# 1879615351/Go-RIO

Hardware: AMD Instinct MI355X
Metric: APD-GICP GN iters/sec on 16k-pt scans + GP-preint windows/sec (higher is better)
Workload: dtype f32 search / f64 accumulate; 1 GPU; C4: 64 scan pairs 16384x16384 + 64 GP windows 1 s @ 200 Hz per GPU, k-NN covariances + 20 fixed GN iterations per pair; pairs_per_gpu=64, target_points=16384, optimizer=GN (convergence test disabled), search=pruned, parallelism=batch shard x1 (no collective)

## Files before the change

go-rio_amd/apd.py:

```python
import ctypes as C
import os

import numpy as np

REG_NONE, REG_MIN_EIG, REG_NORMALIZED_MIN_EIG, REG_PLANE, REG_FROBENIUS = range(5)
OPT_GAUSS_NEWTON, OPT_LEVENBERG_MARQUARDT = 0, 1
SEARCH_BRUTE_FORCE, SEARCH_PRUNED = 0, 1


class GorioError(RuntimeError):
    def __init__(self, code, msg):
        super().__init__(f"gorio error {code}: {msg}")
        self.code = code


class ApdParams(C.Structure):

    _fields_ = [
        ("k_correspondences", C.c_int),
        ("regularization", C.c_int),
        ("dist_var", C.c_double),
        ("azimuth_var", C.c_double),
        ("elevation_var", C.c_double),
        ("corr_dist_threshold", C.c_double),
        ("max_iterations", C.c_int),
        ("rotation_epsilon", C.c_double),
        ("transformation_epsilon", C.c_double),
        ("optimizer", C.c_int),
        ("lm_max_iterations", C.c_int),
        ("lm_init_lambda_factor", C.c_double),
        ("search", C.c_int),
        ("cl_weight_points", C.c_int),
        ("keep_knn_indices", C.c_int),
    ]


APD_SYMBOLS = [
    "gorio_apd_create", "gorio_apd_destroy", "gorio_apd_last_error", "gorio_apd_default_params", "gorio_apd_set_params",
    "gorio_apd_get_params", "gorio_apd_set_source", "gorio_apd_set_target", "gorio_apd_set_source_device",
    "gorio_apd_set_target_device", "gorio_apd_set_clouds_device_batch", "gorio_apd_clear_source", "gorio_apd_clear_target", "gorio_apd_swap_source_and_target",
    "gorio_apd_set_source_covariances", "gorio_apd_set_target_covariances", "gorio_apd_get_source_covariances",
    "gorio_apd_get_target_covariances", "gorio_apd_calculate_covariances", "gorio_apd_get_knn_indices", "gorio_apd_align",
    "gorio_apd_align_batch", "gorio_apd_linearize", "gorio_apd_compute_error", "gorio_apd_get_correspondences",
    "gorio_apd_get_mahalanobis", "gorio_apd_transform_source", "gorio_apd_fitness_score", "gorio_apd_fitness_score_batch", "gorio_apd_set_profiling",
    "gorio_apd_get_stage_times", "gorio_apd_set_target_shared", "gorio_comm_get_unique_id", "gorio_apd_comm_init", "gorio_apd_comm_destroy", "gorio_apd_comm_info", "gorio_apd_debug_set_shard", "gorio_apd_debug_set_schedule", "gorio_apd_set_target_submap", "gorio_apd_get_target_points",
    "gorio_apd_set_method", "gorio_apd_get_method", "gorio_apd_get_voxelmap", "gorio_apd_get_voxel_correspondences",
]

METHOD_APDGICP, METHOD_GICP, METHOD_VGICP = 0, 1, 2
VOXEL_DIRECT27, VOXEL_DIRECT7, VOXEL_DIRECT1, VOXEL_DIRECT_RADIUS = 0, 1, 2, 3
VOXEL_ADDITIVE, VOXEL_ADDITIVE_WEIGHTED, VOXEL_MULTIPLICATIVE = 0, 1, 2
VOXEL_OFFSETS = {VOXEL_DIRECT27: 27, VOXEL_DIRECT7: 7, VOXEL_DIRECT1: 1}

_lib = None


def load_library():
    global _lib
    if _lib is None:
        from . import LIB_PATH

        if not os.path.exists(LIB_PATH):
            raise GorioError(-2, f"{LIB_PATH} is missing: run __graft_entry__.build() (no CPU fallback exists)")
        _lib = C.CDLL(LIB_PATH)
        _lib.gorio_apd_last_error.restype = C.c_char_p
    return _lib


def _p(a, t):
    return C.cast(a.__array_interface__["data"][0], C.POINTER(t))


def _check(h, rc):
    if rc < 0:
        msg = load_library().gorio_apd_last_error(h)
        raise GorioError(rc, msg.decode() if msg else "")
    return rc

# ... 189 lines not shown

    def clearTarget(self):
        _check(self._h, self._lib.gorio_apd_clear_target(self._h))
        self._n_tgt = 0

    def swapSourceAndTarget(self):
        _check(self._h, self._lib.gorio_apd_swap_source_and_target(self._h))
        self._n_src, self._n_tgt = self._n_tgt, self._n_src

    def setSourceCovariances(self, cov):
        cov = np.ascontiguousarray(cov, np.float64).reshape(-1, 16)
        _check(self._h, self._lib.gorio_apd_set_source_covariances(self._h, _p(cov, C.c_double), cov.shape[0]))

    def setTargetCovariances(self, cov):
        cov = np.ascontiguousarray(cov, np.float64).reshape(-1, 16)
        _check(self._h, self._lib.gorio_apd_set_target_covariances(self._h, _p(cov, C.c_double), cov.shape[0]))

    def _get_covs(self, fn, n):
        cnt = _check(self._h, fn(self._h, None, 0))
        out = np.zeros((cnt, 4, 4), np.float64)
        if cnt:
            _check(self._h, fn(self._h, _p(out, C.c_double), cnt))
        return out

    def getSourceCovariances(self):
        return self._get_covs(self._lib.gorio_apd_get_source_covariances, self._n_src)

    def getTargetCovariances(self):
        return self._get_covs(self._lib.gorio_apd_get_target_covariances, self._n_tgt)

    def calculateCovariances(self):
        _check(self._h, self._lib.gorio_apd_calculate_covariances(self._h))

    def getKnnIndices(self, which):
        n = self._n_src if which == 0 else self._n_tgt
        k = self.params.k_correspondences
        idx = np.empty((n, k), np.int32)
        _check(self._h, self._lib.gorio_apd_get_knn_indices(self._h, int(which), _p(idx, C.c_int), n * k))
        return idx

    def align(self, guess=None):
        g = np.ascontiguousarray(np.eye(4) if guess is None else guess, np.float32)
        T = np.zeros((4, 4), np.float32)
        H = np.zeros((6, 6), np.float64)
        conv, nit, nlin = C.c_int(0), C.c_int(0), C.c_int(0)
        _check(self._h, self._lib.gorio_apd_align(self._h, _p(g, C.c_float), _p(T, C.c_float), _p(H, C.c_double), C.byref(conv), C.byref(nit), C.byref(nlin)))
        self._final = T
        self._converged = bool(conv.value)
        return dict(T=T, H=H, converged=bool(conv.value), nr_iterations=nit.value, n_linearize=nlin.value)

    def hasConverged(self):
        return self._converged

    def getFinalTransformation(self):
        return self._final

    def linearize(self, T):
        T = np.ascontiguousarray(T, np.float64)
        H = np.zeros((6, 6), np.float64)
        b = np.zeros(6, np.float64)
        err = C.c_double(0.0)
        _check(self._h, self._lib.gorio_apd_linearize(self._h, _p(T, C.c_double), _p(H, C.c_double), _p(b, C.c_double), C.byref(err)))
        return err.value, H, b

    def evaluateCost(self, relative_pose):
        return self.linearize(np.asarray(relative_pose, np.float32).astype(np.float64))
# ... 112 lines not shown
```

go-rio_amd/csrc/apd_api.hip:

```cpp
#include <hip/hip_runtime.h>
#include <dlfcn.h>
#include <rccl/rccl.h>

#include <cfloat>
#include <climits>
#include <cmath>
#include <cstdio>
#include <cstdlib>
#include <cstring>
#include <memory>
#include <mutex>
#include <string>
#include <unordered_set>
#include <vector>

#include "../../include/gorio_apd.h"
#include "apd_kernels.hip"
#include "apd_index.hip"
#include "apd_submap.hip"
#include "apd_voxel.hip"
#include "apd_prep.hip"
#include "../../include/gorio_prep.h"
#include "apd_ground.hip"
#include "../../include/gorio_sc.h"
#include "apd_sc.hip"

using namespace gorio;

namespace {

constexpr int kPad = 16;
constexpr float kFar = 1e30f;

struct DevCloud {
  float *x = nullptr, *y = nullptr, *z = nullptr, *label = nullptr;
  float4* p4 = nullptr;
  double *cov6 = nullptr, *geo_w = nullptr;
  int* knn = nullptr;
  int* redo = nullptr;
  float* kth = nullptr;
  int redo_cap = 0;
  float* part_d = nullptr;
  int* part_i = nullptr;
  size_t part_cap = 0;
  int knn_k = 0;
  bool knn_valid = false;
  int n = 0, n_pad = 0, cap = 0;
  bool present = false;
  int cov_count = 0;
  int cov_k = -1, cov_reg = -1;
  SearchIndex idx = SearchIndex{nullptr, nullptr, nullptr, nullptr, nullptr, nullptr, nullptr, nullptr, 0, 0, 0, 0};
  unsigned long long* keys = nullptr;
  unsigned int* bb = nullptr;
  int idx_cap = 0, keys_cap = 0;
  bool idx_valid = false;
  unsigned long long* vm_keys = nullptr;
  int vm_keys_cap = 0;
  int* vm_counts = nullptr;
  int vm_counts_cap = 0;
  int* vm_bb = nullptr;
  IndexJob* vm_job = nullptr;
  unsigned long long* vm_vkey = nullptr;
  double* vm_mean = nullptr;
  double* vm_cov6 = nullptr;
  int* vm_num = nullptr;
  int vm_cap = 0, vm_nv = 0;
  int vm_min[3] = {0, 0, 0}, vm_dim[3] = {0, 0, 0};
  double vm_res = 0.0;
  bool vm_mult = false;
  bool vm_valid = false;
  VoxelMapView voxel_view() const { return VoxelMapView{vm_vkey, vm_mean, vm_cov6, vm_num, vm_nv, {vm_min[0], vm_min[1], vm_min[2]}, {vm_dim[0], vm_dim[1], vm_dim[2]}, vm_res}; }
  int device = 0;
  CloudView view() const { return CloudView{x, y, z, label, p4, cov6, geo_w, n, n_pad, idx}; }
  DevCloud() = default;
  DevCloud(const DevCloud&) = delete;
  DevCloud& operator=(const DevCloud&) = delete;
  ~DevCloud();
};

}

struct gorio_apd {
  int device = 0;
  hipStream_t stream = nullptr;
  gorio_apd_params params;
  std::shared_ptr<DevCloud> src, tgt;
  unsigned long long* best_key = nullptr;
  int* seed = nullptr;
// ... 393 lines not shown
      HIP_TRY(h, hipMalloc(&c.idx.s4, sizeof(float4) * cap));
      HIP_TRY(h, hipMalloc(&c.idx.tbox, sizeof(float) * 8 * (cap / 32)));
      HIP_TRY(h, hipMalloc(&c.idx.sbox, sizeof(float) * 8 * (cap / 512)));
      HIP_TRY(h, hipMalloc(&c.idx.bbox, sizeof(float) * 8 * (cap / 32768 + 1)));
      c.idx_cap = cap;
    }
    if (npow2 > c.keys_cap) {
      hipFree(c.keys);
      c.keys = nullptr;
      HIP_TRY(h, hipMalloc(&c.keys, sizeof(unsigned long long) * npow2));
      c.keys_cap = npow2;
    }
    if (!c.bb) HIP_TRY(h, hipMalloc(&c.bb, sizeof(unsigned int) * 6));
    c.idx.n = c.n;
    c.idx.n_spad = n_spad;
    c.idx.n_tiles = n_spad / 32;
    c.idx.n_super = n_spad / 512;
    IndexJob& j = jobs[q];
    j.x = c.x; j.y = c.y; j.z = c.z; j.n = c.n; j.npow2 = npow2; j.keys = c.keys; j.bb = c.bb; j.idx = c.idx;
    max_pow2 = std::max(max_pow2, npow2);
    max_spad = std::max(max_spad, n_spad);
    max_n = std::max(max_n, c.n);
  }
  if (nj > lead->ijobs_cap) {
    hipFree(lead->d_ijobs);
    lead->d_ijobs = nullptr;
    HIP_TRY(lead, hipMalloc(&lead->d_ijobs, sizeof(IndexJob) * nj));
    lead->ijobs_cap = nj;
  }
  if (int rc = upload_staged(lead, lead->pin_ijobs, lead->d_ijobs, jobs.data(), sizeof(IndexJob) * nj)) return rc;
  {
    StageTimer t(lead, 4);
    const IndexJob* dj = lead->d_ijobs;
    bbox_init_kernel<<<(nj + 63) / 64, 64, 0, lead->stream>>>(dj, nj);
    bbox_kernel<<<dim3(std::min(64, (max_n + 255) / 256), nj), 256, 0, lead->stream>>>(dj);
    morton_kernel<<<dim3((max_pow2 + 255) / 256, nj), 256, 0, lead->stream>>>(dj);
    bitonic_tile_sort_kernel<<<dim3(max_pow2 / kSortTile, nj), 1024, 0, lead->stream>>>(dj);
    for (int k = 2 * kSortTile; k <= max_pow2; k <<= 1) {
      for (int j = k >> 1; j >= kSortTile; j >>= 1) bitonic_global_kernel<<<dim3((max_pow2 / 2 + 255) / 256, nj), 256, 0, lead->stream>>>(dj, k, j);
      bitonic_tile_merge_kernel<<<dim3(max_pow2 / kSortTile, nj), 1024, 0, lead->stream>>>(dj, k);
    }
    gather_sorted_kernel<<<dim3((max_spad + 255) / 256, nj), 256, 0, lead->stream>>>(dj);
    if (small_call) kd_refine_kernel<2048><<<dim3((max_spad + 2047) / 2048, nj), 512, 0, lead->stream>>>(dj);
    else kd_refine_kernel<4096><<<dim3((max_spad + 4095) / 4096, nj), 1024, 0, lead->stream>>>(dj);
    box_tile_kernel<<<dim3((max_spad / 32 + 255) / 256, nj), 256, 0, lead->stream>>>(dj);
    box_super_kernel<<<dim3((max_spad / 512 + 255) / 256, nj), 256, 0, lead->stream>>>(dj);
    box_block_kernel<<<dim3((max_spad / 32768 + 64) / 64, nj), 64, 0, lead->stream>>>(dj);
  }
  HIP_TRY(lead, hipGetLastError());
  for (auto& t : todo) t.second->idx_valid = true;
  return GORIO_OK;
}

int run_covariances(gorio_apd* lead, std::vector<std::pair<gorio_apd*, DevCloud*>>& todo) {
  if (todo.empty()) return GORIO_OK;
  const int njobs = (int)todo.size();
  const int k = lead->params.k_correspondences;
  const int K = k <= 20 ? 20 : 32;
  const bool pruned = lead->params.search == GORIO_SEARCH_PRUNED;
  const bool select = pruned && K == 20;
  if (pruned) {
    int rc = run_index_build(lead, todo);
    if (rc) return rc;
  }
  long total_waves = 0;
  int max_n = 0;
  for (auto& t : todo) {
    total_waves += (t.second->n + 63) / 64;
    if (t.second->n > max_n) max_n = t.second->n;
  }
  int splits = (int)((8192 + total_waves - 1) / total_waves);
  if (splits < 1) splits = 1;
  if (splits > 32) splits = 32;
  if (pruned) splits = 1;
  std::vector<KnnJob> jobs(njobs);
  int max_splits = 1;
  for (int q = 0; q < njobs; ++q) {
    gorio_apd* h = todo[q].first;
    DevCloud& c = *todo[q].second;
    int chunk = roundup((c.n_pad + splits - 1) / splits, kPad);
    if (chunk < 256) chunk = 256;
    const int s = pruned ? 1 : (c.n_pad + chunk - 1) / chunk;
    if (s > max_splits) max_splits = s;
// ... 1465 lines not shown
  h->shard_only = false;
  h->corr_valid = false;
  return GORIO_OK;
}

int gorio_apd_comm_info(gorio_apd_t* h, int* world_size, int* rank, long long* allreduce_count) {
  if (!h) return GORIO_ERR_INVALID;
  if (!h->comm) return fail(h, GORIO_ERR_STATE, "comm_info: the handle has no communicator");
  Rccl& R = rccl();
  int w = 0, r = 0;
  if (!R.CommCount || !R.CommUserRank) return fail(h, GORIO_ERR_NO_DEVICE, "librccl lacks ncclCommCount / ncclCommUserRank");
  NCCL_TRY(h, R.CommCount(h->comm, &w));
  NCCL_TRY(h, R.CommUserRank(h->comm, &r));
  if (world_size) *world_size = w;
  if (rank) *rank = r;
  if (allreduce_count) *allreduce_count = h->allreduce_count;
  return GORIO_OK;
}

int gorio_apd_debug_set_shard(gorio_apd_t* h, int world_size, int rank) {
  if (!h || world_size < 1 || rank < 0 || rank >= world_size) return GORIO_ERR_INVALID;
  if (h->comm) return fail(h, GORIO_ERR_STATE, "debug_set_shard: the handle has a communicator");
  h->comm_world = world_size;
  h->comm_rank = rank;
  h->shard_only = world_size > 1;
  h->corr_valid = false;
  return GORIO_OK;
}

int gorio_apd_debug_set_schedule(gorio_apd_t* h, int fuse_step, int plan_search) {
  if (!h) return GORIO_ERR_INVALID;
  h->fuse_step = fuse_step != 0;
  h->plan_search = plan_search != 0;
  return GORIO_OK;
}

int gorio_apd_comm_destroy(gorio_apd_t* h) {
  if (!h) return GORIO_ERR_INVALID;
  if (h->comm) {
    hipSetDevice(h->device);
    hipStreamSynchronize(h->stream);
    if (rccl().ok) rccl().CommDestroy(h->comm);
    h->comm = nullptr;
  }
  h->comm_world = 1;
  h->comm_rank = 0;
  h->shard_only = false;
  h->corr_valid = false;
  return GORIO_OK;
}

int gorio_apd_set_profiling(gorio_apd_t* h, int enable) {
  if (!h) return GORIO_ERR_INVALID;
  h->profiling = enable != 0;
  for (int i = 0; i < 8; ++i) { h->stage_s[i] = 0; h->stage_n[i] = 0; }
  return GORIO_OK;
}

int gorio_apd_get_stage_times(gorio_apd_t* h, double seconds[8], int counts[8]) {
  if (!h) return GORIO_ERR_INVALID;
  for (int i = 0; i < 8; ++i) {
    if (seconds) seconds[i] = h->stage_s[i];
    if (counts) counts[i] = h->stage_n[i];
  }
  return GORIO_OK;
}
// ... 595 lines not shown
```

go-rio_amd/csrc/apd_index.hip:

```cpp
#include <hip/hip_runtime.h>

namespace gorio {

__device__ __forceinline__ unsigned int f2ord(float f) {
  const unsigned int u = __float_as_uint(f);
  return (u & 0x80000000u) ? ~u : (u | 0x80000000u);
}
__device__ __forceinline__ float ord2f(unsigned int o) {
  const unsigned int u = (o & 0x80000000u) ? (o & 0x7fffffffu) : ~o;
  return __uint_as_float(u);
}

__global__ void bbox_init_kernel(const IndexJob* __restrict__ jobs, int nj) {
  const int q = blockIdx.x * 64 + threadIdx.x;
  if (q >= nj) return;
  for (int a = 0; a < 3; ++a) {
    jobs[q].bb[a] = 0xffffffffu;
    jobs[q].bb[3 + a] = 0u;
  }
}

__global__ __launch_bounds__(256) void bbox_kernel(const IndexJob* __restrict__ jobs) {
  const IndexJob& jb = jobs[blockIdx.y];
  float lo[3] = {INFINITY, INFINITY, INFINITY}, hi[3] = {-INFINITY, -INFINITY, -INFINITY};
  for (int i = blockIdx.x * 256 + threadIdx.x; i < jb.n; i += gridDim.x * 256) {
    const float v[3] = {jb.x[i], jb.y[i], jb.z[i]};
#pragma unroll
    for (int a = 0; a < 3; ++a) {
      lo[a] = fminf(lo[a], v[a]);
      hi[a] = fmaxf(hi[a], v[a]);
    }
  }
#pragma unroll
  for (int a = 0; a < 3; ++a) {
#pragma unroll
    for (int off = 32; off > 0; off >>= 1) {
      lo[a] = fminf(lo[a], __shfl_down(lo[a], off, 64));
      hi[a] = fmaxf(hi[a], __shfl_down(hi[a], off, 64));
    }
    if ((threadIdx.x & 63) == 0) {
      atomicMin(jb.bb + a, f2ord(lo[a]));
      atomicMax(jb.bb + 3 + a, f2ord(hi[a]));
    }
  }
}

__device__ __forceinline__ unsigned long long spread11(unsigned int v) {
  unsigned long long x = v & 0x7ffu;
  x = (x | (x << 32)) & 0x1f00000000ffffull;
  x = (x | (x << 16)) & 0x1f0000ff0000ffull;
  x = (x | (x << 8)) & 0x100f00f00f00f00full;
  x = (x | (x << 4)) & 0x10c30c30c30c30c3ull;
  x = (x | (x << 2)) & 0x1249249249249249ull;
  return x;
}

__global__ __launch_bounds__(256) void morton_kernel(const IndexJob* __restrict__ jobs) {
  const IndexJob& jb = jobs[blockIdx.y];
  const int i = blockIdx.x * 256 + threadIdx.x;
  if (i >= jb.npow2) return;
  unsigned long long key = ~0ull;
  if (i < jb.n) {
    unsigned int q[3];
    const float v[3] = {jb.x[i], jb.y[i], jb.z[i]};
    float ext = 1e-6f;
#pragma unroll
    for (int a = 0; a < 3; ++a) ext = fmaxf(ext, ord2f(jb.bb[3 + a]) - ord2f(jb.bb[a]));
#pragma unroll
    for (int a = 0; a < 3; ++a) {
      const float lo = ord2f(jb.bb[a]);
      float t = (v[a] - lo) / ext * 2047.0f;
      t = fminf(fmaxf(t, 0.0f), 2047.0f);
      q[a] = (unsigned int)t;
    }
    const unsigned long long code = spread11(q[0]) | (spread11(q[1]) << 1) | (spread11(q[2]) << 2);
    key = (code << 31) | (unsigned long long)i;
  }
  jb.keys[i] = key;
}

constexpr int kSortTile = 4096;

__device__ __forceinline__ void cmpx(unsigned long long& a, unsigned long long& b, bool up) {
  if ((a > b) == up) {
    const unsigned long long t = a;
    a = b;
    b = t;
  }
}

__global__ __launch_bounds__(1024) void bitonic_tile_sort_kernel(const IndexJob* __restrict__ jobs) {
  const IndexJob& jb = jobs[blockIdx.y];
  const int base = blockIdx.x * kSortTile;
  if (base >= jb.npow2) return;
  __shared__ unsigned long long s[kSortTile];
  for (int q = threadIdx.x; q < kSortTile; q += 1024) s[q] = jb.keys[base + q];
  __syncthreads();
  for (int k = 2; k <= kSortTile; k <<= 1) {
    for (int j = k >> 1; j > 0; j >>= 1) {
      for (int t = threadIdx.x; t < kSortTile / 2; t += 1024) {
        const int lo = ((t / j) * 2 * j) + (t % j), hi = lo + j;
        const bool up = (((base + lo) & k) == 0);
        unsigned long long a = s[lo], b = s[hi];
        cmpx(a, b, up);
        s[lo] = a;
        s[hi] = b;
      }
      __syncthreads();
    }
  }
  for (int q = threadIdx.x; q < kSortTile; q += 1024) jb.keys[base + q] = s[q];
// ... 5 lines not shown
  const int t = blockIdx.x * 256 + threadIdx.x;
  if (t >= jb.npow2 / 2) return;
  const int lo = ((t / j) * 2 * j) + (t % j), hi = lo + j;
  const bool up = ((lo & k) == 0);
  unsigned long long a = jb.keys[lo], b = jb.keys[hi];
  if ((a > b) == up) {
    jb.keys[lo] = b;
    jb.keys[hi] = a;
  }
}

__global__ __launch_bounds__(1024) void bitonic_tile_merge_kernel(const IndexJob* __restrict__ jobs, int k) {
  const IndexJob& jb = jobs[blockIdx.y];
  if (k > jb.npow2) return;
  const int base = blockIdx.x * kSortTile;
  if (base >= jb.npow2) return;
  __shared__ unsigned long long s[kSortTile];
  for (int q = threadIdx.x; q < kSortTile; q += 1024) s[q] = jb.keys[base + q];
  __syncthreads();
  for (int j = kSortTile >> 1; j > 0; j >>= 1) {
    for (int t = threadIdx.x; t < kSortTile / 2; t += 1024) {
      const int lo = ((t / j) * 2 * j) + (t % j), hi = lo + j;
      const bool up = (((base + lo) & k) == 0);
      unsigned long long a = s[lo], b = s[hi];
      cmpx(a, b, up);
      s[lo] = a;
      s[hi] = b;
    }
    __syncthreads();
  }
  for (int q = threadIdx.x; q < kSortTile; q += 1024) jb.keys[base + q] = s[q];
}

__global__ __launch_bounds__(256) void gather_sorted_kernel(const IndexJob* __restrict__ jobs) {
  const IndexJob& jb = jobs[blockIdx.y];
  const int p = blockIdx.x * 256 + threadIdx.x;
  if (p >= jb.idx.n_spad) return;
  if (p < jb.n) {
    const int i = (int)(jb.keys[p] & 0x7fffffffull);
    jb.idx.sx[p] = jb.x[i];
    jb.idx.sy[p] = jb.y[i];
    jb.idx.sz[p] = jb.z[i];
    jb.idx.orig[p] = i;
    jb.idx.s4[p] = make_float4(jb.x[i], jb.y[i], jb.z[i], __int_as_float(i));
  } else {
    jb.idx.sx[p] = 1e30f;
    jb.idx.sy[p] = 1e30f;
    jb.idx.sz[p] = 1e30f;
    jb.idx.orig[p] = 0x7fffffff;
    jb.idx.s4[p] = make_float4(1e30f, 1e30f, 1e30f, __int_as_float(0x7fffffff));
  }
}

constexpr int kKdSmallCloud = 131072;
template <int kKdChunk>
__global__ __launch_bounds__(kKdChunk / 4) void kd_refine_kernel(const IndexJob* __restrict__ jobs) {
  constexpr int kKdThreads = kKdChunk / 4;
  const IndexJob& jb = jobs[blockIdx.y];
  const int base = blockIdx.x * kKdChunk;
  if (base >= jb.idx.n_spad) return;
  __shared__ float px[kKdChunk], py[kKdChunk], pz[kKdChunk];
  __shared__ int po[kKdChunk];
  __shared__ unsigned long long keys[kKdChunk];
  __shared__ unsigned int sb[64][6];
  const int tid = threadIdx.x, lane = tid & 63;
  for (int e = tid; e < kKdChunk; e += kKdThreads) {
    const int p = base + e;
    const bool in = p < jb.idx.n_spad;
    px[e] = in ? jb.idx.sx[p] : 1e30f;
    py[e] = in ? jb.idx.sy[p] : 1e30f;
    pz[e] = in ? jb.idx.sz[p] : 1e30f;
    po[e] = in ? jb.idx.orig[p] : 0x7fffffff;
  }
  __syncthreads();
  for (int seg = kKdChunk; seg >= 64; seg >>= 1) {
    const int nseg = kKdChunk / seg;
    for (int q = tid; q < nseg * 6; q += kKdThreads) sb[q / 6][q % 6] = (q % 6) < 3 ? 0xffffffffu : 0u;
    __syncthreads();
    for (int r = 0; r < 4; ++r) {
      const int e = tid + kKdThreads * r;
      const bool valid = po[e] != 0x7fffffff;
      const float v[3] = {px[e], py[e], pz[e]};
#pragma unroll
      for (int a = 0; a < 3; ++a) {
        unsigned int lo = valid ? f2ord(v[a]) : 0xffffffffu, hi = valid ? f2ord(v[a]) : 0u;
#pragma unroll
        for (int off = 32; off > 0; off >>= 1) {
          lo = min(lo, (unsigned int)__shfl_xor((int)lo, off, 64));
          hi = max(hi, (unsigned int)__shfl_xor((int)hi, off, 64));
        }
        if (lane == 0) {
          atomicMin(&sb[e / seg][a], lo);
          atomicMax(&sb[e / seg][3 + a], hi);
        }
      }
    }
    __syncthreads();
    for (int r = 0; r < 4; ++r) {
      const int e = tid + kKdThreads * r;
      const unsigned int* b = sb[e / seg];
      int axis = 0;
      float best = -1.0f;
#pragma unroll
      for (int a = 0; a < 3; ++a) {
        const float ext = b[3 + a] >= b[a] ? ord2f(b[3 + a]) - ord2f(b[a]) : 0.0f;
        if (ext > best) {
          best = ext;
          axis = a;
        }
      }
      const float c = axis == 0 ? px[e] : (axis == 1 ? py[e] : pz[e]);
      keys[e] = ((unsigned long long)f2ord(c) << 12) | (unsigned long long)e;
    }
    __syncthreads();
    for (int lk = 1; (1 << lk) <= seg; ++lk) {
      const int k = 1 << lk;
      int lj = lk - 1;
      for (; lj >= 8; --lj) {
        const int j = 1 << lj;
        for (int r = 0; r < 2; ++r) {
          const int t = tid + kKdThreads * r;
          const int lo = ((t >> lj) << (lj + 1)) | (t & (j - 1)), hi = lo + j;
          const bool up = (k == seg) || ((lo & k) == 0);
          unsigned long long a = keys[lo], b = keys[hi];
          if ((a > b) == up) {
            keys[lo] = b;
            keys[hi] = a;
          }
        }
        __syncthreads();
      }
      const int wbase = (tid >> 6) * 256;
      for (; lj >= 0; --lj) {
        const int j = 1 << lj;
        for (int r = 0; r < 2; ++r) {
          const int t = lane + 64 * r;
          const int lo = wbase + (((t >> lj) << (lj + 1)) | (t & (j - 1))), hi = lo + j;
          const bool up = (k == seg) || ((lo & k) == 0);
          unsigned long long a = keys[lo], b = keys[hi];
          if ((a > b) == up) {
            keys[lo] = b;
            keys[hi] = a;
          }
        }
        __builtin_amdgcn_fence(__ATOMIC_RELEASE, "wavefront");
        __builtin_amdgcn_wave_barrier();
        __builtin_amdgcn_fence(__ATOMIC_ACQUIRE, "wavefront");
      }
      if (k >= 256 && 2 * k <= seg) __syncthreads();
    }
    __syncthreads();
    float nx[4], ny[4], nz[4];
    int no[4];
    for (int r = 0; r < 4; ++r) {
      const int src = (int)(keys[tid + kKdThreads * r] & 4095ull);
      nx[r] = px[src]; ny[r] = py[src]; nz[r] = pz[src]; no[r] = po[src];
    }
    __syncthreads();
    for (int r = 0; r < 4; ++r) {
      const int e = tid + kKdThreads * r;
      px[e] = nx[r]; py[e] = ny[r]; pz[e] = nz[r]; po[e] = no[r];
    }
    __syncthreads();
  }
  for (int e = tid; e < kKdChunk; e += kKdThreads) {
    const int p = base + e;
    if (p < jb.idx.n_spad) {
      jb.idx.sx[p] = px[e];
      jb.idx.sy[p] = py[e];
      jb.idx.sz[p] = pz[e];
      jb.idx.orig[p] = po[e];
      jb.idx.s4[p] = make_float4(px[e], py[e], pz[e], __int_as_float(po[e]));
    }
  }
}

__global__ __launch_bounds__(256) void box_tile_kernel(const IndexJob* __restrict__ jobs) {
  const IndexJob& jb = jobs[blockIdx.y];
  const int t = blockIdx.x * 256 + threadIdx.x;
  if (t >= jb.idx.n_tiles) return;
  float lo[3] = {INFINITY, INFINITY, INFINITY}, hi[3] = {-INFINITY, -INFINITY, -INFINITY};
  for (int q = 0; q < 32; ++q) {
    const int p = t * 32 + q;
    if (p < jb.n) {
      const float v[3] = {jb.idx.sx[p], jb.idx.sy[p], jb.idx.sz[p]};
#pragma unroll
      for (int a = 0; a < 3; ++a) {
        lo[a] = fminf(lo[a], v[a]);
        hi[a] = fmaxf(hi[a], v[a]);
      }
    }
  }
  float* b = jb.idx.tbox + (size_t)t * 8;
  b[0] = lo[0]; b[1] = lo[1]; b[2] = lo[2]; b[3] = 0.f;
  b[4] = hi[0]; b[5] = hi[1]; b[6] = hi[2]; b[7] = 0.f;
}
__global__ __launch_bounds__(256) void box_super_kernel(const IndexJob* __restrict__ jobs) {
  const IndexJob& jb = jobs[blockIdx.y];
  const int s = blockIdx.x * 256 + threadIdx.x;
  if (s >= jb.idx.n_super) return;
  float lo[3] = {INFINITY, INFINITY, INFINITY}, hi[3] = {-INFINITY, -INFINITY, -INFINITY};
  for (int q = 0; q < 16; ++q) {
    const int t = s * 16 + q;
    if (t < jb.idx.n_tiles) {
      const float* b = jb.idx.tbox + (size_t)t * 8;
#pragma unroll
      for (int a = 0; a < 3; ++a) {
        lo[a] = fminf(lo[a], b[a]);
        hi[a] = fmaxf(hi[a], b[4 + a]);
      }
    }
  }
  float* b = jb.idx.sbox + (size_t)s * 8;
  b[0] = lo[0]; b[1] = lo[1]; b[2] = lo[2]; b[3] = 0.f;
  b[4] = hi[0]; b[5] = hi[1]; b[6] = hi[2]; b[7] = 0.f;
}

__global__ __launch_bounds__(64) void box_block_kernel(const IndexJob* __restrict__ jobs) {
  const IndexJob& jb = jobs[blockIdx.y];
  const int k = blockIdx.x * 64 + threadIdx.x;
  if (k >= (jb.idx.n_super + 63) / 64) return;
  float lo[3] = {INFINITY, INFINITY, INFINITY}, hi[3] = {-INFINITY, -INFINITY, -INFINITY};
  for (int q = 0; q < 64; ++q) {
    const int t = k * 64 + q;
    if (t < jb.idx.n_super) {
      const float* b = jb.idx.sbox + (size_t)t * 8;
#pragma unroll
      for (int a = 0; a < 3; ++a) {
        lo[a] = fminf(lo[a], b[a]);
        hi[a] = fmaxf(hi[a], b[4 + a]);
      }
    }
  }
  float* b = jb.idx.bbox + (size_t)k * 8;
  b[0] = lo[0]; b[1] = lo[1]; b[2] = lo[2]; b[3] = 0.f;
  b[4] = hi[0]; b[5] = hi[1]; b[6] = hi[2]; b[7] = 0.f;
}


__device__ __forceinline__ float box_bound(float qx, float qy, float qz, const float* __restrict__ b) {
  const float cx = fminf(fmaxf(qx, b[0]), b[4]);
  const float cy = fminf(fmaxf(qy, b[1]), b[5]);
  const float cz = fminf(fmaxf(qz, b[2]), b[6]);
  const float dx = qx - cx, dy = qy - cy, dz = qz - cz;
  float r = dx * dx;
  r = r + dy * dy;
  r = r + dz * dz;
  return r;
// ... 784 lines not shown
```

include/gorio_apd.h:

```cpp
#ifndef GORIO_APD_H
#define GORIO_APD_H

#ifdef __cplusplus
extern "C" {
#endif

typedef enum {
  GORIO_OK = 0,
  GORIO_ERR_INVALID = -1,
  GORIO_ERR_NO_DEVICE = -2,
  GORIO_ERR_STATE = -3,
  GORIO_ERR_ALLOC = -4,
  GORIO_ERR_UNSUPPORTED = -5
} gorio_status;

typedef enum { GORIO_REG_NONE = 0, GORIO_REG_MIN_EIG = 1, GORIO_REG_NORMALIZED_MIN_EIG = 2, GORIO_REG_PLANE = 3, GORIO_REG_FROBENIUS = 4 } gorio_regularization;
typedef enum { GORIO_OPT_GAUSS_NEWTON = 0, GORIO_OPT_LEVENBERG_MARQUARDT = 1 } gorio_optimizer;
typedef enum { GORIO_SEARCH_BRUTE_FORCE = 0, GORIO_SEARCH_PRUNED = 1 } gorio_search;

typedef enum { GORIO_METHOD_APDGICP = 0, GORIO_METHOD_GICP = 1, GORIO_METHOD_VGICP = 2 } gorio_method;
typedef enum { GORIO_VOXEL_DIRECT27 = 0, GORIO_VOXEL_DIRECT7 = 1, GORIO_VOXEL_DIRECT1 = 2, GORIO_VOXEL_DIRECT_RADIUS = 3 } gorio_voxel_search;
typedef enum { GORIO_VOXEL_ADDITIVE = 0, GORIO_VOXEL_ADDITIVE_WEIGHTED = 1, GORIO_VOXEL_MULTIPLICATIVE = 2 } gorio_voxel_mode;

typedef struct {
// ... 57 lines not shown

int gorio_apd_clear_source(gorio_apd_t* h);
int gorio_apd_clear_target(gorio_apd_t* h);
int gorio_apd_swap_source_and_target(gorio_apd_t* h);

int gorio_apd_set_source_covariances(gorio_apd_t* h, const double* cov4x4, int n);
int gorio_apd_set_target_covariances(gorio_apd_t* h, const double* cov4x4, int n);
int gorio_apd_get_source_covariances(gorio_apd_t* h, double* cov4x4, int n);
int gorio_apd_get_target_covariances(gorio_apd_t* h, double* cov4x4, int n);
int gorio_apd_calculate_covariances(gorio_apd_t* h);
int gorio_apd_get_knn_indices(gorio_apd_t* h, int which, int* idx, int n_times_k);

int gorio_apd_align(gorio_apd_t* h, const float guess[16], float T_out[16], double* H_out, int* converged, int* nr_iterations, int* n_linearize);

int gorio_apd_align_batch(gorio_apd_t** handles, int count, const float* guesses, float* T_out, double* H_out, int* converged, int* nr_iterations, int* n_linearize);

int gorio_apd_linearize(gorio_apd_t* h, const double T[16], double* H, double* b, double* error);
int gorio_apd_compute_error(gorio_apd_t* h, const double T[16], double* error);
int gorio_apd_get_correspondences(gorio_apd_t* h, int* corr, float* sq_dist, int n);
int gorio_apd_get_mahalanobis(gorio_apd_t* h, double* maha4x4, int n);

int gorio_apd_transform_source(gorio_apd_t* h, const float T[16], float* xyz_out, int n, int point_stride_bytes);

int gorio_apd_fitness_score(gorio_apd_t* h, const float T[16], double max_range, double inlier_dist, double* score, double* inlier_fraction);

int gorio_apd_fitness_score_batch(gorio_apd_t** handles, int count, const float* T, double max_range, double inlier_dist, double* score, double* inlier_fraction);

int gorio_comm_get_unique_id(char id[128]);
int gorio_apd_comm_init(gorio_apd_t* h, int world_size, int rank, const char id[128]);
int gorio_apd_comm_destroy(gorio_apd_t* h);
int gorio_apd_comm_info(gorio_apd_t* h, int* world_size, int* rank, long long* allreduce_count);
int gorio_apd_debug_set_shard(gorio_apd_t* h, int world_size, int rank);
int gorio_apd_debug_set_schedule(gorio_apd_t* h, int fuse_step, int plan_search);

int gorio_apd_set_profiling(gorio_apd_t* h, int enable);
int gorio_apd_get_stage_times(gorio_apd_t* h, double seconds[8], int counts[8]);

#ifdef __cplusplus
}
#endif
#endif
```

Before: 162,900 linearisations/s.

## Fuse search-index build kernels and skip redundant kd-split sorts

Rebuilds the pruned-search index construction. Clouds up to 32k points get one fused bbox+Morton kernel in place of three launches. The sorted-gather step is folded into kd_refine, which now reads the Morton-sorted keys directly. The tile and super-box reductions also move into kd_refine, using shared memory and wave shuffles. In addition, kd segments whose split axis matches the parent's skip their bitonic sort. A debug readback API for the index is added. This cuts launches and global memory round trips in the per-pair index build. The risks are a single 1024-thread block per cloud doing the bbox pass serially, and that skipping sorts relies on the parent split leaving the child already ordered.

```diff
diff --git a/go-rio_amd/apd.py b/go-rio_amd/apd.py
--- a/go-rio_amd/apd.py
+++ b/go-rio_amd/apd.py
@@ -43,7 +43,7 @@
     "gorio_apd_get_target_covariances", "gorio_apd_calculate_covariances", "gorio_apd_get_knn_indices", "gorio_apd_align",
     "gorio_apd_align_batch", "gorio_apd_linearize", "gorio_apd_compute_error", "gorio_apd_get_correspondences",
     "gorio_apd_get_mahalanobis", "gorio_apd_transform_source", "gorio_apd_fitness_score", "gorio_apd_fitness_score_batch", "gorio_apd_set_profiling",
-    "gorio_apd_get_stage_times", "gorio_apd_set_target_shared", "gorio_comm_get_unique_id", "gorio_apd_comm_init", "gorio_apd_comm_destroy", "gorio_apd_comm_info", "gorio_apd_debug_set_shard", "gorio_apd_debug_set_schedule", "gorio_apd_set_target_submap", "gorio_apd_get_target_points",
+    "gorio_apd_get_stage_times", "gorio_apd_set_target_shared", "gorio_comm_get_unique_id", "gorio_apd_comm_init", "gorio_apd_comm_destroy", "gorio_apd_comm_info", "gorio_apd_debug_set_shard", "gorio_apd_debug_set_schedule", "gorio_apd_debug_get_index", "gorio_apd_set_target_submap", "gorio_apd_get_target_points",
     "gorio_apd_set_method", "gorio_apd_get_method", "gorio_apd_get_voxelmap", "gorio_apd_get_voxel_correspondences",
 ]
 
@@ -299,6 +299,17 @@
     def calculateCovariances(self):
         _check(self._h, self._lib.gorio_apd_calculate_covariances(self._h))
 
+    def debugGetIndex(self, which):
+        sizes = (C.c_int * 6)()
+        _check(self._h, self._lib.gorio_apd_debug_get_index(self._h, int(which), sizes, None, None, None, None, None))
+        n, n_spad, n_tiles, n_super, n_blk, chunk = list(sizes)
+        sxyz = np.empty(7 * n_spad, np.float32)
+        orig = np.empty(n_spad, np.int32)
+        tbox, sbox, bbox = (np.empty((m, 8), np.float32) for m in (n_tiles, n_super, n_blk))
+        _check(self._h, self._lib.gorio_apd_debug_get_index(self._h, int(which), sizes, _p(sxyz, C.c_float), _p(orig, C.c_int), _p(tbox, C.c_float), _p(sbox, C.c_float), _p(bbox, C.c_float)))
+        return dict(n=n, n_spad=n_spad, kd_chunk=chunk, sx=sxyz[:n_spad], sy=sxyz[n_spad : 2 * n_spad], sz=sxyz[2 * n_spad : 3 * n_spad],
+                    s4=sxyz[3 * n_spad :].reshape(n_spad, 4), orig=orig, tbox=tbox, sbox=sbox, bbox=bbox)
+
     def getKnnIndices(self, which):
         n = self._n_src if which == 0 else self._n_tgt
         k = self.params.k_correspondences
diff --git a/go-rio_amd/csrc/apd_api.hip b/go-rio_amd/csrc/apd_api.hip
--- a/go-rio_amd/csrc/apd_api.hip
+++ b/go-rio_amd/csrc/apd_api.hip
@@ -54,6 +54,7 @@
   unsigned int* bb = nullptr;
   int idx_cap = 0, keys_cap = 0;
   bool idx_valid = false;
+  int idx_chunk = 0;
   unsigned long long* vm_keys = nullptr;
   int vm_keys_cap = 0;
   int* vm_counts = nullptr;
@@ -513,23 +514,27 @@
   {
     StageTimer t(lead, 4);
     const IndexJob* dj = lead->d_ijobs;
-    bbox_init_kernel<<<(nj + 63) / 64, 64, 0, lead->stream>>>(dj, nj);
-    bbox_kernel<<<dim3(std::min(64, (max_n + 255) / 256), nj), 256, 0, lead->stream>>>(dj);
-    morton_kernel<<<dim3((max_pow2 + 255) / 256, nj), 256, 0, lead->stream>>>(dj);
+    if (max_n <= kBboxFusedMax) {
+      bbox_morton_kernel<<<nj, 1024, 0, lead->stream>>>(dj);
+    } else {
+      bbox_init_kernel<<<(nj + 63) / 64, 64, 0, lead->stream>>>(dj, nj);
+      bbox_kernel<<<dim3(std::min(64, (max_n + 255) / 256), nj), 256, 0, lead->stream>>>(dj);
+      morton_kernel<<<dim3((max_pow2 + 255) / 256, nj), 256, 0, lead->stream>>>(dj);
+    }
     bitonic_tile_sort_kernel<<<dim3(max_pow2 / kSortTile, nj), 1024, 0, lead->stream>>>(dj);
     for (int k = 2 * kSortTile; k <= max_pow2; k <<= 1) {
       for (int j = k >> 1; j >= kSortTile; j >>= 1) bitonic_global_kernel<<<dim3((max_pow2 / 2 + 255) / 256, nj), 256, 0, lead->stream>>>(dj, k, j);
       bitonic_tile_merge_kernel<<<dim3(max_pow2 / kSortTile, nj), 1024, 0, lead->stream>>>(dj, k);
     }
-    gather_sorted_kernel<<<dim3((max_spad + 255) / 256, nj), 256, 0, lead->stream>>>(dj);
     if (small_call) kd_refine_kernel<2048><<<dim3((max_spad + 2047) / 2048, nj), 512, 0, lead->stream>>>(dj);
     else kd_refine_kernel<4096><<<dim3((max_spad + 4095) / 4096, nj), 1024, 0, lead->stream>>>(dj);
-    box_tile_kernel<<<dim3((max_spad / 32 + 255) / 256, nj), 256, 0, lead->stream>>>(dj);
-    box_super_kernel<<<dim3((max_spad / 512 + 255) / 256, nj), 256, 0, lead->stream>>>(dj);
     box_block_kernel<<<dim3((max_spad / 32768 + 64) / 64, nj), 64, 0, lead->stream>>>(dj);
   }
   HIP_TRY(lead, hipGetLastError());
-  for (auto& t : todo) t.second->idx_valid = true;
+  for (auto& t : todo) {
+    t.second->idx_valid = true;
+    t.second->idx_chunk = small_call ? 2048 : 4096;
+  }
   return GORIO_OK;
 }
 
@@ -2061,6 +2066,28 @@
   if (!h) return GORIO_ERR_INVALID;
   h->fuse_step = fuse_step != 0;
   h->plan_search = plan_search != 0;
+  return GORIO_OK;
+}
+
+int gorio_apd_debug_get_index(gorio_apd_t* h, int which, int sizes[6], float* sxyz, int* orig, float* tbox, float* sbox, float* bbox) {
+  if (!h || !sizes) return GORIO_ERR_INVALID;
+  DevCloud& c = which == 0 ? *h->src : *h->tgt;
+  if (!c.present || !c.idx_valid) return fail(h, GORIO_ERR_STATE, "debug_get_index: no search index held for this cloud (pruned search, after the covariances or a linearisation)");
+  const SearchIndex& ix = c.idx;
+  const int n_blk = (ix.n_super + 63) / 64;
+  sizes[0] = ix.n; sizes[1] = ix.n_spad; sizes[2] = ix.n_tiles; sizes[3] = ix.n_super; sizes[4] = n_blk; sizes[5] = c.idx_chunk;
+  HIP_TRY(h, hipSetDevice(h->device));
+  HIP_TRY(h, hipStreamSynchronize(h->stream));
+  if (sxyz) {
+    HIP_TRY(h, hipMemcpy(sxyz, ix.sx, sizeof(float) * ix.n_spad, hipMemcpyDeviceToHost));
+    HIP_TRY(h, hipMemcpy(sxyz + ix.n_spad, ix.sy, sizeof(float) * ix.n_spad, hipMemcpyDeviceToHost));
+    HIP_TRY(h, hipMemcpy(sxyz + 2 * (size_t)ix.n_spad, ix.sz, sizeof(float) * ix.n_spad, hipMemcpyDeviceToHost));
+    HIP_TRY(h, hipMemcpy(sxyz + 3 * (size_t)ix.n_spad, ix.s4, sizeof(float4) * ix.n_spad, hipMemcpyDeviceToHost));
+  }
+  if (orig) HIP_TRY(h, hipMemcpy(orig, ix.orig, sizeof(int) * ix.n_spad, hipMemcpyDeviceToHost));
+  if (tbox) HIP_TRY(h, hipMemcpy(tbox, ix.tbox, sizeof(float) * 8 * ix.n_tiles, hipMemcpyDeviceToHost));
+  if (sbox) HIP_TRY(h, hipMemcpy(sbox, ix.sbox, sizeof(float) * 8 * ix.n_super, hipMemcpyDeviceToHost));
+  if (bbox) HIP_TRY(h, hipMemcpy(bbox, ix.bbox, sizeof(float) * 8 * n_blk, hipMemcpyDeviceToHost));
   return GORIO_OK;
 }
 
diff --git a/go-rio_amd/csrc/apd_index.hip b/go-rio_amd/csrc/apd_index.hip
--- a/go-rio_amd/csrc/apd_index.hip
+++ b/go-rio_amd/csrc/apd_index.hip
@@ -55,28 +55,81 @@
   return x;
 }
 
+__device__ __forceinline__ unsigned long long morton_key(const IndexJob& jb, int i, const float (&lo)[3], float ext) {
+  if (i >= jb.n) return ~0ull;
+  unsigned int q[3];
+  const float v[3] = {jb.x[i], jb.y[i], jb.z[i]};
+#pragma unroll
+  for (int a = 0; a < 3; ++a) {
+    float t = (v[a] - lo[a]) / ext * 2047.0f;
+    t = fminf(fmaxf(t, 0.0f), 2047.0f);
+    q[a] = (unsigned int)t;
+  }
+  const unsigned long long code = spread11(q[0]) | (spread11(q[1]) << 1) | (spread11(q[2]) << 2);
+  return (code << 31) | (unsigned long long)i;
+}
+
 __global__ __launch_bounds__(256) void morton_kernel(const IndexJob* __restrict__ jobs) {
   const IndexJob& jb = jobs[blockIdx.y];
   const int i = blockIdx.x * 256 + threadIdx.x;
   if (i >= jb.npow2) return;
-  unsigned long long key = ~0ull;
-  if (i < jb.n) {
-    unsigned int q[3];
+  float ext = 1e-6f, lo[3];
+#pragma unroll
+  for (int a = 0; a < 3; ++a) {
+    lo[a] = ord2f(jb.bb[a]);
+    ext = fmaxf(ext, ord2f(jb.bb[3 + a]) - lo[a]);
+  }
+  jb.keys[i] = morton_key(jb, i, lo, ext);
+}
+
+constexpr int kBboxFusedMax = 32768;
+__global__ __launch_bounds__(1024) void bbox_morton_kernel(const IndexJob* __restrict__ jobs) {
+  const IndexJob& jb = jobs[blockIdx.x];
+  __shared__ unsigned int s_bb[16][6];
+  const int tid = threadIdx.x;
+  float flo[3] = {INFINITY, INFINITY, INFINITY}, fhi[3] = {-INFINITY, -INFINITY, -INFINITY};
+  for (int i = tid; i < jb.n; i += 1024) {
     const float v[3] = {jb.x[i], jb.y[i], jb.z[i]};
-    float ext = 1e-6f;
-#pragma unroll
-    for (int a = 0; a < 3; ++a) ext = fmaxf(ext, ord2f(jb.bb[3 + a]) - ord2f(jb.bb[a]));
 #pragma unroll
     for (int a = 0; a < 3; ++a) {
-      const float lo = ord2f(jb.bb[a]);
-      float t = (v[a] - lo) / ext * 2047.0f;
-      t = fminf(fmaxf(t, 0.0f), 2047.0f);
-      q[a] = (unsigned int)t;
-    }
-    const unsigned long long code = spread11(q[0]) | (spread11(q[1]) << 1) | (spread11(q[2]) << 2);
-    key = (code << 31) | (unsigned long long)i;
-  }
-  jb.keys[i] = key;
+      flo[a] = fminf(flo[a], v[a]);
+      fhi[a] = fmaxf(fhi[a], v[a]);
+    }
+  }
+#pragma unroll
+  for (int a = 0; a < 3; ++a) {
+#pragma unroll
+    for (int off = 32; off > 0; off >>= 1) {
+      flo[a] = fminf(flo[a], __shfl_xor(flo[a], off, 64));
+      fhi[a] = fmaxf(fhi[a], __shfl_xor(fhi[a], off, 64));
+    }
+    if ((tid & 63) == 0) {
+      s_bb[tid >> 6][a] = f2ord(flo[a]);
+      s_bb[tid >> 6][3 + a] = f2ord(fhi[a]);
+    }
+  }
+  __syncthreads();
+  unsigned int bb[6];
+#pragma unroll
+  for (int a = 0; a < 3; ++a) {
+    bb[a] = 0xffffffffu;
+    bb[3 + a] = 0u;
+    for (int w = 0; w < 16; ++w) {
+      bb[a] = min(bb[a], s_bb[w][a]);
+      bb[3 + a] = max(bb[3 + a], s_bb[w][3 + a]);
+    }
+  }
+  if (tid == 0) {
+#pragma unroll
+    for (int a = 0; a < 6; ++a) jb.bb[a] = bb[a];
+  }
+  float ext = 1e-6f, lo[3];
+#pragma unroll
+  for (int a = 0; a < 3; ++a) {
+    lo[a] = ord2f(bb[a]);
+    ext = fmaxf(ext, ord2f(bb[3 + a]) - lo[a]);
+  }
+  for (int i = tid; i < jb.npow2; i += 1024) jb.keys[i] = morton_key(jb, i, lo, ext);
 }
 
 constexpr int kSortTile = 4096;
@@ -148,30 +201,14 @@
   for (int q = threadIdx.x; q < kSortTile; q += 1024) jb.keys[base + q] = s[q];
 }
 
-__global__ __launch_bounds__(256) void gather_sorted_kernel(const IndexJob* __restrict__ jobs) {
-  const IndexJob& jb = jobs[blockIdx.y];
-  const int p = blockIdx.x * 256 + threadIdx.x;
-  if (p >= jb.idx.n_spad) return;
-  if (p < jb.n) {
-    const int i = (int)(jb.keys[p] & 0x7fffffffull);
-    jb.idx.sx[p] = jb.x[i];
-    jb.idx.sy[p] = jb.y[i];
-    jb.idx.sz[p] = jb.z[i];
-    jb.idx.orig[p] = i;
-    jb.idx.s4[p] = make_float4(jb.x[i], jb.y[i], jb.z[i], __int_as_float(i));
-  } else {
-    jb.idx.sx[p] = 1e30f;
-    jb.idx.sy[p] = 1e30f;
-    jb.idx.sz[p] = 1e30f;
-    jb.idx.orig[p] = 0x7fffffff;
-    jb.idx.s4[p] = make_float4(1e30f, 1e30f, 1e30f, __int_as_float(0x7fffffff));
-  }
-}
-
+#ifndef GORIO_KD_SKIP_SORTED
+#define GORIO_KD_SKIP_SORTED 1
+#endif
 constexpr int kKdSmallCloud = 131072;
 template <int kKdChunk>
 __global__ __launch_bounds__(kKdChunk / 4) void kd_refine_kernel(const IndexJob* __restrict__ jobs) {
   constexpr int kKdThreads = kKdChunk / 4;
+  constexpr int kTiles = kKdChunk / 32, kSupers = kKdChunk / 512;
   const IndexJob& jb = jobs[blockIdx.y];
   const int base = blockIdx.x * kKdChunk;
   if (base >= jb.idx.n_spad) return;
@@ -179,19 +216,26 @@
   __shared__ int po[kKdChunk];
   __shared__ unsigned long long keys[kKdChunk];
   __shared__ unsigned int sb[64][6];
+  __shared__ int sax[2][64];
+  __shared__ int sskip[64];
+  __shared__ int s_nsort;
+  __shared__ float tb[kTiles][6];
   const int tid = threadIdx.x, lane = tid & 63;
   for (int e = tid; e < kKdChunk; e += kKdThreads) {
     const int p = base + e;
-    const bool in = p < jb.idx.n_spad;
-    px[e] = in ? jb.idx.sx[p] : 1e30f;
-    py[e] = in ? jb.idx.sy[p] : 1e30f;
-    pz[e] = in ? jb.idx.sz[p] : 1e30f;
-    po[e] = in ? jb.idx.orig[p] : 0x7fffffff;
+    const bool in = p < jb.n;
+    const int i = in ? (int)(jb.keys[p] & 0x7fffffffull) : 0;
+    px[e] = in ? jb.x[i] : 1e30f;
+    py[e] = in ? jb.y[i] : 1e30f;
+    pz[e] = in ? jb.z[i] : 1e30f;
+    po[e] = in ? i : 0x7fffffff;
   }
   __syncthreads();
-  for (int seg = kKdChunk; seg >= 64; seg >>= 1) {
+  int lseg = __builtin_ctz(kKdChunk), cur = 0;
+  for (int seg = kKdChunk; seg >= 64; seg >>= 1, --lseg, cur ^= 1) {
     const int nseg = kKdChunk / seg;
     for (int q = tid; q < nseg * 6; q += kKdThreads) sb[q / 6][q % 6] = (q % 6) < 3 ? 0xffffffffu : 0u;
+    if (tid == 0) s_nsort = 0;
     __syncthreads();
     for (int r = 0; r < 4; ++r) {
       const int e = tid + kKdThreads * r;
@@ -212,9 +256,8 @@
       }
     }
     __syncthreads();
-    for (int r = 0; r < 4; ++r) {
-      const int e = tid + kKdThreads * r;
-      const unsigned int* b = sb[e / seg];
+    if (tid < nseg) {
+      const unsigned int* b = sb[tid];
       int axis = 0;
       float best = -1.0f;
 #pragma unroll
@@ -225,10 +268,23 @@
           axis = a;
         }
       }
+      const bool skip = GORIO_KD_SKIP_SORTED && seg != kKdChunk && sax[cur ^ 1][tid >> 1] == axis;
+      sax[cur][tid] = axis;
+      sskip[tid] = skip ? 1 : 0;
+      if (!skip) s_nsort = 1;
+    }
+    __syncthreads();
+    if (s_nsort == 0) continue;
+    for (int r = 0; r < 4; ++r) {
+      const int e = tid + kKdThreads * r;
+      const int axis = sax[cur][e >> lseg];
       const float c = axis == 0 ? px[e] : (axis == 1 ? py[e] : pz[e]);
       keys[e] = ((unsigned long long)f2ord(c) << 12) | (unsigned long long)e;
     }
     __syncthreads();
+    const int wbase = (tid >> 6) * 256;
+    bool wskip = true;
+    for (int q = wbase >> lseg; q <= (wbase + 255) >> lseg; ++q) wskip = wskip && sskip[q] != 0;
     for (int lk = 1; (1 << lk) <= seg; ++lk) {
       const int k = 1 << lk;
       int lj = lk - 1;
@@ -237,6 +293,7 @@
         for (int r = 0; r < 2; ++r) {
           const int t = tid + kKdThreads * r;
           const int lo = ((t >> lj) << (lj + 1)) | (t & (j - 1)), hi = lo + j;
+          if (sskip[lo >> lseg]) continue;
           const bool up = (k == seg) || ((lo & k) == 0);
           unsigned long long a = keys[lo], b = keys[hi];
           if ((a > b) == up) {
@@ -246,22 +303,23 @@
         }
         __syncthreads();
       }
-      const int wbase = (tid >> 6) * 256;
-      for (; lj >= 0; --lj) {
-        const int j = 1 << lj;
-        for (int r = 0; r < 2; ++r) {
-          const int t = lane + 64 * r;
-          const int lo = wbase + (((t >> lj) << (lj + 1)) | (t & (j - 1))), hi = lo + j;
-          const bool up = (k == seg) || ((lo & k) == 0);
-          unsigned long long a = keys[lo], b = keys[hi];
-          if ((a > b) == up) {
-            keys[lo] = b;
-            keys[hi] = a;
+      if (!wskip) {
+        for (; lj >= 0; --lj) {
+          const int j = 1 << lj;
+          for (int r = 0; r < 2; ++r) {
+            const int t = lane + 64 * r;
+            const int lo = wbase + (((t >> lj) << (lj + 1)) | (t & (j - 1))), hi = lo + j;
+            const bool up = (k == seg) || ((lo & k) == 0);
+            unsigned long long a = keys[lo], b = keys[hi];
+            if ((a > b) == up) {
+              keys[lo] = b;
+              keys[hi] = a;
+            }
           }
-        }
-        __builtin_amdgcn_fence(__ATOMIC_RELEASE, "wavefront");
-        __builtin_amdgcn_wave_barrier();
-        __builtin_amdgcn_fence(__ATOMIC_ACQUIRE, "wavefront");
+          __builtin_amdgcn_fence(__ATOMIC_RELEASE, "wavefront");
+          __builtin_amdgcn_wave_barrier();
+          __builtin_amdgcn_fence(__ATOMIC_ACQUIRE, "wavefront");
+        }
       }
       if (k >= 256 && 2 * k <= seg) __syncthreads();
     }
@@ -289,47 +347,63 @@
       jb.idx.s4[p] = make_float4(px[e], py[e], pz[e], __int_as_float(po[e]));
     }
   }
-}
-
-__global__ __launch_bounds__(256) void box_tile_kernel(const IndexJob* __restrict__ jobs) {
-  const IndexJob& jb = jobs[blockIdx.y];
-  const int t = blockIdx.x * 256 + threadIdx.x;
-  if (t >= jb.idx.n_tiles) return;
-  float lo[3] = {INFINITY, INFINITY, INFINITY}, hi[3] = {-INFINITY, -INFINITY, -INFINITY};
-  for (int q = 0; q < 32; ++q) {
-    const int p = t * 32 + q;
-    if (p < jb.n) {
-      const float v[3] = {jb.idx.sx[p], jb.idx.sy[p], jb.idx.sz[p]};
+  {
+    const int t = tid >> 3, sub = tid & 7;
+    float lo[3] = {INFINITY, INFINITY, INFINITY}, hi[3] = {-INFINITY, -INFINITY, -INFINITY};
+    for (int r = 0; r < 4; ++r) {
+      const int e = t * 32 + sub + 8 * r;
+      if (base + e < jb.n) {
+        const float v[3] = {px[e], py[e], pz[e]};
+#pragma unroll
+        for (int a = 0; a < 3; ++a) {
+          lo[a] = fminf(lo[a], v[a]);
+          hi[a] = fmaxf(hi[a], v[a]);
+        }
+      }
+    }
+#pragma unroll
+    for (int a = 0; a < 3; ++a) {
+#pragma unroll
+      for (int off = 4; off > 0; off >>= 1) {
+        lo[a] = fminf(lo[a], __shfl_xor(lo[a], off, 64));
+        hi[a] = fmaxf(hi[a], __shfl_xor(hi[a], off, 64));
+      }
+    }
+    if (sub == 0) {
 #pragma unroll
       for (int a = 0; a < 3; ++a) {
-        lo[a] = fminf(lo[a], v[a]);
-        hi[a] = fmaxf(hi[a], v[a]);
-      }
-    }
-  }
-  float* b = jb.idx.tbox + (size_t)t * 8;
-  b[0] = lo[0]; b[1] = lo[1]; b[2] = lo[2]; b[3] = 0.f;
-  b[4] = hi[0]; b[5] = hi[1]; b[6] = hi[2]; b[7] = 0.f;
-}
-__global__ __launch_bounds__(256) void box_super_kernel(const IndexJob* __restrict__ jobs) {
-  const IndexJob& jb = jobs[blockIdx.y];
-  const int s = blockIdx.x * 256 + threadIdx.x;
-  if (s >= jb.idx.n_super) return;
-  float lo[3] = {INFINITY, INFINITY, INFINITY}, hi[3] = {-INFINITY, -INFINITY, -INFINITY};
-  for (int q = 0; q < 16; ++q) {
-    const int t = s * 16 + q;
-    if (t < jb.idx.n_tiles) {
-      const float* b = jb.idx.tbox + (size_t)t * 8;
-#pragma unroll
-      for (int a = 0; a < 3; ++a) {
-        lo[a] = fminf(lo[a], b[a]);
-        hi[a] = fmaxf(hi[a], b[4 + a]);
-      }
-    }
-  }
-  float* b = jb.idx.sbox + (size_t)s * 8;
-  b[0] = lo[0]; b[1] = lo[1]; b[2] = lo[2]; b[3] = 0.f;
-  b[4] = hi[0]; b[5] = hi[1]; b[6] = hi[2]; b[7] = 0.f;
+        tb[t][a] = lo[a];
+        tb[t][3 + a] = hi[a];
+      }
+      const int gt = base / 32 + t;
+      if (gt < jb.idx.n_tiles) {
+        float4* b = reinterpret_cast<float4*>(jb.idx.tbox + (size_t)gt * 8);
+        b[0] = make_float4(lo[0], lo[1], lo[2], 0.f);
+        b[1] = make_float4(hi[0], hi[1], hi[2], 0.f);
+      }
+    }
+  }
+  __syncthreads();
+  if (tid < kSupers * 16) {
+    const int sp = tid >> 4, q = tid & 15;
+    float lo[3], hi[3];
+#pragma unroll
+    for (int a = 0; a < 3; ++a) {
+      lo[a] = tb[sp * 16 + q][a];
+      hi[a] = tb[sp * 16 + q][3 + a];
+#pragma unroll
+      for (int off = 8; off > 0; off >>= 1) {
+        lo[a] = fminf(lo[a], __shfl_xor(lo[a], off, 64));
+        hi[a] = fmaxf(hi[a], __shfl_xor(hi[a], off, 64));
+      }
+    }
+    const int gs = base / 512 + sp;
+    if (q == 0 && gs < jb.idx.n_super) {
+      float4* b = reinterpret_cast<float4*>(jb.idx.sbox + (size_t)gs * 8);
+      b[0] = make_float4(lo[0], lo[1], lo[2], 0.f);
+      b[1] = make_float4(hi[0], hi[1], hi[2], 0.f);
+    }
+  }
 }
 
 __global__ __launch_bounds__(64) void box_block_kernel(const IndexJob* __restrict__ jobs) {
diff --git a/include/gorio_apd.h b/include/gorio_apd.h
--- a/include/gorio_apd.h
+++ b/include/gorio_apd.h
@@ -113,6 +113,7 @@
 int gorio_apd_comm_info(gorio_apd_t* h, int* world_size, int* rank, long long* allreduce_count);
 int gorio_apd_debug_set_shard(gorio_apd_t* h, int world_size, int rank);
 int gorio_apd_debug_set_schedule(gorio_apd_t* h, int fuse_step, int plan_search);
+int gorio_apd_debug_get_index(gorio_apd_t* h, int which, int sizes[6], float* sxyz, int* orig, float* tbox, float* sbox, float* bbox);
 
 int gorio_apd_set_profiling(gorio_apd_t* h, int enable);
 int gorio_apd_get_stage_times(gorio_apd_t* h, double seconds[8], int counts[8]);
```

After: 171,100 linearisations/s, median of 6. +5.1%, better.
